# ChangUk/RecommenderSystems

Hardware: AMD Instinct MI355X
Metric: RWR seeds/sec + achieved HBM GB/s on 100M-edge bipartite graph, 1/2/4/8 GPUs (higher is better)
Workload: dtype f64

## Files before the change

### include/rwr.h

```cpp
#ifndef RWR_H
#define RWR_H

#include <stdint.h>

#ifdef __cplusplus
extern "C" {
#endif

#define RWR_VERSION_STRING "0.4.0"

enum {
    RWR_OK            = 0,
    RWR_E_INVALID     = 1,
    RWR_E_RANGE       = 2,
    RWR_E_NO_DEVICE   = 3,
    RWR_E_HIP         = 4,
    RWR_E_NOMEM       = 5,
    RWR_E_CAPACITY    = 6,
    RWR_E_UNSUPPORTED = 7
};

enum { RWR_NODE_UNDEFINED = 0, RWR_NODE_USER = 1, RWR_NODE_ITEM = 2, RWR_NODE_ETC = 3 };
enum { RWR_EDGE_UNDEFINED = 0, RWR_EDGE_LIKE = 1, RWR_EDGE_FRIENDSHIP = 2, RWR_EDGE_FOLLOW = 3,
       RWR_EDGE_MENTION = 4, RWR_EDGE_AUTHORSHIP = 5, RWR_EDGE_PURCHASE = 6, RWR_EDGE_ETC = 7 };
// ... 16 lines not shown
    int32_t reserved0;
} rwr_opts;

typedef struct rwr_stats {
    int32_t struct_size;
    int32_t n;
    int64_t nnz_raw;
    int64_t nnz;
    int32_t uniform;
    int32_t tile_seeds;
    int32_t tile_group;
    int32_t mode;
    double  build_ms;
    double  spmm_ms;
    int64_t spmm_launches;
    int64_t spmm_seed_steps;
    double  chain_ms;
    int64_t chain_launches;
    double  rank_ms;
    double  iterate_wall_ms;
    double  total_wall_ms;
    int64_t seeds_done;
    int64_t chain_redo_blocks;
    double  spmm_dense_ms;
    int64_t spmm_dense_launches;
    int64_t spmm_dense_seed_steps;
    int32_t uniform_path;
    int32_t reserved1;
    int64_t frontier_list_launches;
    int64_t rank_fused_groups;
    int64_t rank_fused_fallbacks;
    int64_t rank_pruned_rows;
    double  rank_bound_ms;
} rwr_stats;


const char *rwr_version(void);
int32_t rwr_device_count(void);
const char *rwr_last_error(void);

int32_t rwr_graph_create(int32_t n, const int64_t *node_id, const uint8_t *node_type,
                         const int64_t *rowptr , const int32_t *dst, const uint8_t *etype,
                         const double *w, const rwr_opts *opts , rwr_graph **out);
int32_t rwr_graph_destroy(rwr_graph *g);
int32_t rwr_graph_update_links(rwr_graph *g, int64_t count, const int64_t *link_index,
                               const uint8_t *etype , const double *w );
int32_t rwr_graph_append_links(rwr_graph *g, int64_t count, const int32_t *src, const int32_t *dst,
                               const uint8_t *etype, const double *w,
                               int64_t *new_index_out );
int32_t rwr_graph_size(const rwr_graph *g, int32_t *n, int64_t *nnz_raw, int64_t *nnz_explicit);
int32_t rwr_graph_get_normalized(rwr_graph *g, double *w_out , uint8_t *dangling_out );

int32_t rwr_recommend(rwr_graph *g, int32_t seed, float d, int32_t n_iter, int32_t top_n,
                      int64_t *out_id, double *out_score, int64_t *inout_count);

int32_t rwr_recommend_eval(rwr_graph *g, int32_t seed, float d, int32_t n_iter, const int64_t *test_ids,
                           int64_t n_test, int64_t *n_hits, double *sum_precision, int64_t *list_len);

int32_t rwr_recommend_eval_batch(rwr_graph *g, const int32_t *seeds, int32_t K, float d, int32_t n_iter,
                                 const int64_t *test_ptr, const int64_t *test_ids, int64_t *n_hits,
                                 double *sum_precision, int64_t *list_len);

typedef struct rwr_graph_desc {
    int32_t n_nodes;
    int32_t reserved0;
    const int64_t *node_id;
// ... 47 lines not shown
```

### recommendersystems_amd/_lib.py

```python
from __future__ import annotations

import ctypes as C
import os

_HERE = os.path.dirname(os.path.abspath(__file__))
LIB_PATH = os.path.join(_HERE, "librwr.so")

RWR_OK, RWR_E_INVALID, RWR_E_RANGE, RWR_E_NO_DEVICE, RWR_E_HIP, RWR_E_NOMEM, RWR_E_CAPACITY, RWR_E_UNSUPPORTED = range(8)
RWR_MODE_EXACT = 0
RWR_RUN_ITERATIONS, RWR_RUN_THRESHOLD, RWR_RUN_DEFAULT_THRESHOLD = 0, 1, 2

EXPORTS = [
    "rwr_version", "rwr_device_count", "rwr_last_error",
    "rwr_graph_create", "rwr_graph_update_links", "rwr_graph_append_links", "rwr_graph_destroy", "rwr_graph_size", "rwr_graph_get_normalized",
    "rwr_recommend", "rwr_recommend_eval", "rwr_recommend_eval_batch", "rwr_eval_graphs", "rwr_recommend_batch", "rwr_model_run", "rwr_model_deliver",
    "rwr_model_run_restart", "rwr_model_deliver_restart", "rwr_model_run_batch", "rwr_model_run_restart_batch",
    "rwr_recommend_restart_batch",
    "rwr_part_begin", "rwr_part_step", "rwr_part_local_step", "rwr_part_finish_step", "rwr_part_rank",
    "rwr_get_stats", "rwr_reset_stats",
]


class rwr_opts(C.Structure):
    _fields_ = [("struct_size", C.c_int32), ("device", C.c_int32), ("mode", C.c_int32),
                ("tile_seeds", C.c_int32), ("tile_group", C.c_int32), ("profile", C.c_int32),
                ("workspace_bytes", C.c_int64), ("seed_row_kernel", C.c_int32), ("reserved0", C.c_int32)]


class rwr_graph_desc(C.Structure):
    _fields_ = [("n_nodes", C.c_int32), ("reserved0", C.c_int32), ("node_id", C.POINTER(C.c_int64)),
                ("node_type", C.POINTER(C.c_uint8)), ("rowptr", C.POINTER(C.c_int64)), ("dst", C.POINTER(C.c_int32)),
                ("etype", C.POINTER(C.c_uint8)), ("w", C.POINTER(C.c_double))]


class rwr_stats(C.Structure):
    _fields_ = [("struct_size", C.c_int32), ("n", C.c_int32), ("nnz_raw", C.c_int64), ("nnz", C.c_int64),
                ("uniform", C.c_int32), ("tile_seeds", C.c_int32), ("tile_group", C.c_int32), ("mode", C.c_int32),
                ("build_ms", C.c_double), ("spmm_ms", C.c_double), ("spmm_launches", C.c_int64),
                ("spmm_seed_steps", C.c_int64), ("chain_ms", C.c_double), ("chain_launches", C.c_int64),
                ("rank_ms", C.c_double), ("iterate_wall_ms", C.c_double), ("total_wall_ms", C.c_double),
                ("seeds_done", C.c_int64), ("chain_redo_blocks", C.c_int64),
                ("spmm_dense_ms", C.c_double), ("spmm_dense_launches", C.c_int64), ("spmm_dense_seed_steps", C.c_int64),
                ("uniform_path", C.c_int32), ("reserved1", C.c_int32), ("frontier_list_launches", C.c_int64),
                ("rank_fused_groups", C.c_int64), ("rank_fused_fallbacks", C.c_int64),
                ("rank_pruned_rows", C.c_int64), ("rank_bound_ms", C.c_double)]


class RwrError(RuntimeError):
    def __init__(self, status: int, message: str):
        super().__init__(f"librwr status {status}: {message}")
        self.status = status


_lib = None


def load():
    global _lib
    if _lib is not None:
        return _lib
    if not os.path.exists(LIB_PATH):
        raise ImportError(f"{LIB_PATH} not found: build it with `python -c 'import __graft_entry__ as g; g.build()'` "
                          "(hipcc --offload-arch=gfx950); there is no CPU fallback")
    lib = C.CDLL(LIB_PATH)
    p = C.POINTER
    lib.rwr_version.restype = C.c_char_p
    lib.rwr_last_error.restype = C.c_char_p
    lib.rwr_device_count.restype = C.c_int32
    lib.rwr_graph_create.restype = C.c_int32
    lib.rwr_graph_create.argtypes = [C.c_int32, p(C.c_int64), p(C.c_uint8), p(C.c_int64), p(C.c_int32),
                                     p(C.c_uint8), p(C.c_double), p(rwr_opts), p(C.c_void_p)]
    lib.rwr_graph_update_links.restype = C.c_int32
    lib.rwr_graph_update_links.argtypes = [C.c_void_p, C.c_int64, p(C.c_int64), p(C.c_uint8), p(C.c_double)]
    lib.rwr_graph_append_links.restype = C.c_int32
    lib.rwr_graph_append_links.argtypes = [C.c_void_p, C.c_int64, p(C.c_int32), p(C.c_int32), p(C.c_uint8), p(C.c_double),
                                           p(C.c_int64)]
    lib.rwr_graph_destroy.restype = C.c_int32
    lib.rwr_graph_destroy.argtypes = [C.c_void_p]
# ... 62 lines not shown
```

### recommendersystems_amd/csrc/api.hip

```cpp
#include <stdarg.h>
#include <algorithm>
#include <cmath>
#include <mutex>
#include <vector>
#include <stdlib.h>
#include <string.h>

#include "engine.h"
#include "exclude_plan.h"

namespace rwr {

static thread_local char g_err[512] = "";

void set_error(const char *fmt, ...)
{
    va_list ap;
    va_start(ap, fmt);
    vsnprintf(g_err, sizeof(g_err), fmt, ap);
    va_end(ap);
}

static int usable_devices()
{
// ... 954 lines not shown
}

int32_t rwr_part_rank(rwr_graph *g, void *dev_x, int32_t top_n, int64_t *ids, double *scores, int32_t *counts)
{
    g_err[0] = 0;
    if (!g || !dev_x || !ids || !scores || !counts) { set_error("rwr_part_rank: NULL argument"); return RWR_E_INVALID; }
    RWR_BIND(g);
    return part_rank(g, (double *)dev_x, top_n, ids, scores, counts);
}

int32_t rwr_get_stats(rwr_graph *g, rwr_stats *out)
{
    if (!g || !out) { set_error("rwr_get_stats: NULL argument"); return RWR_E_INVALID; }
    size_t sz = out->struct_size > 0 ? (size_t)out->struct_size : sizeof(rwr_stats);
    if (sz > sizeof(rwr_stats)) sz = sizeof(rwr_stats);
    rwr_stats s = g->stats;
    s.struct_size = (int32_t)sz;
    memcpy(out, &s, sz);
    return RWR_OK;
}

int32_t rwr_reset_stats(rwr_graph *g)
{
    if (!g) { set_error("rwr_reset_stats: NULL argument"); return RWR_E_INVALID; }
    rwr_stats &s = g->stats;
    s.spmm_ms = s.chain_ms = s.rank_ms = s.iterate_wall_ms = s.total_wall_ms = 0;
    s.spmm_launches = s.spmm_seed_steps = s.chain_launches = s.seeds_done = s.chain_redo_blocks = 0;
    s.spmm_dense_ms = 0;
    s.spmm_dense_launches = s.spmm_dense_seed_steps = 0;
    s.frontier_list_launches = 0;
    s.rank_fused_groups = s.rank_fused_fallbacks = 0;
    s.rank_pruned_rows = 0;
    s.rank_bound_ms = 0;
    return RWR_OK;
}

}
```

### recommendersystems_amd/csrc/iterate.hip

```cpp
#include "iterate.h"

#include <climits>
#include <cstdlib>
#include <type_traits>

namespace rwr {

template <int G, bool VF>
__global__ __launch_bounds__(256) void k_spmm(int32_t n, const int64_t *__restrict__ in_ptr,
                                              const int32_t *__restrict__ in_src,
                                              const double *__restrict__ in_w,
                                              const int32_t *__restrict__ row_order, int32_t nrows,
                                              const double *__restrict__ X, double *__restrict__ Y,
                                              const int32_t *__restrict__ seeds, double c1, int skip_seed_row,
                                              const double *__restrict__ w_src, double *__restrict__ Zout)
{
    constexpr int RPW = WAVE / G;
    constexpr int U = 4;
    const int tile = blockIdx.y;
    const size_t toff = (size_t)tile * (size_t)n * G;
    X += toff;
    Y += toff;
    if (VF && Zout) Zout += toff;
    const int lane = threadIdx.x & (WAVE - 1);
// ... 405 lines not shown
    double acc = 0.0;
    for (size_t w0 = 0; w0 < nzw; w0 += WAVE) {
        const uint32_t word = (w0 + lane < nzw) ? bits[w0 + lane] : 0u;
        unsigned long long mask = __ballot(word != 0u);
        while (mask) {
            const int l = __builtin_ctzll(mask);
            mask &= mask - 1;
            uint32_t wv = (uint32_t)__builtin_amdgcn_readlane((int)word, l);
            while (wv) {
                const int b = __builtin_ctz(wv);
                wv &= wv - 1;
                const int32_t i = (int32_t)((w0 + l) * 32 + b);
                if (consumer && s >= 0) {
                    while (p < e && in_src[p] < i) ++p;
                    while (p < e && in_src[p] == i) { acc += termp[p]; ++p; }
                    const double xi = x[(size_t)i * G + k];
                    const double rw = c1 * xi;
                    acc += dangling[i] ? xi : (xi - rw);
                }
            }
        }
    }
    if (consumer && s >= 0) {
        Y[(size_t)tile * (size_t)n * G + (size_t)s * G + k] = acc;
        if (nz_out && acc != 0.0)
            atomicOr(&nz_out[(size_t)tile * nzw + ((uint32_t)s >> 5)], 1u << (s & 31));
    }
}

constexpr int CH3_NSW = 6;
constexpr int CH3_NST = CH3_NSW * WAVE;
constexpr int CH3_LPT = 16;
constexpr int CH3_CE = CH3_NST * CH3_LPT;
template <int G>
__global__ __launch_bounds__(WAVE + CH3_NST) void k_seed_chain_roles(
    int32_t n, const int64_t *__restrict__ in_ptr, const int32_t *__restrict__ in_src,
    const uint8_t *__restrict__ dangling, const double *__restrict__ X, double *__restrict__ Y,
    const int32_t *__restrict__ seeds, double c1, const int64_t *__restrict__ evoff,
    const double *__restrict__ evterm, uint32_t *__restrict__ nz_out, unsigned int *__restrict__ gate)
{
    if (threadIdx.x == 0 && gate) __hip_atomic_fetch_add(gate, 1u, __ATOMIC_RELAXED, __HIP_MEMORY_SCOPE_AGENT);
    constexpr int CR = CH3_CE / G;
    static_assert(CR % 32 == 0, "chunk rows must be a multiple of 32");
    extern __shared__ double rr[];
    const int tile = blockIdx.x;
    const double *x = X + (size_t)tile * (size_t)n * G;
    const int tid = threadIdx.x;
    const int64_t total = (int64_t)n * G;
    const int nchunks = (int)((total + CH3_CE - 1) / CH3_CE);

    if (tid >= WAVE) {
        const int st = tid - WAVE;
        double rega[CH3_LPT], regb[CH3_LPT];
        uint8_t dga[CH3_LPT], dgb[CH3_LPT];
#define CH3_LOAD(R, D, C)                                                       \
    {                                                                           \
        const int64_t base__ = (int64_t)(C) * CH3_CE;                           \
        _Pragma("unroll") for (int u = 0; u < CH3_LPT; ++u) {                   \
            int64_t el = base__ + (int64_t)u * CH3_NST + st;                    \
            el = el < total ? el : total - 1;                                   \
            R[u] = x[el];                                                       \
            D[u] = dangling[el / G];                                            \
        }                                                                       \
    }
#define CH3_STAGE(R, D, C)                                                                              \
    {                                                                                                   \
        const int64_t base__ = (int64_t)(C) * CH3_CE;                                                   \
        double *buf__ = rr + (size_t)((C) & 1) * CH3_CE;                                                \
        _Pragma("unroll") for (int u = 0; u < CH3_LPT; ++u) {                                           \
            const int off = u * CH3_NST + st;                                                           \
            const double xv = (base__ + off < total) ? R[u] : 0.0;   \
            const double rw = c1 * xv;                                                                  \
            buf__[off] = D[u] ? xv : (xv - rw);                                                         \
        }                                                                                               \
    }
        CH3_LOAD(rega, dga, 0)
        if (nchunks > 1) CH3_LOAD(regb, dgb, 1)
        for (int c = 0; c < nchunks; c += 2) {
            CH3_STAGE(rega, dga, c)
            if (c + 2 < nchunks) CH3_LOAD(rega, dga, c + 2)
            __builtin_amdgcn_fence(__ATOMIC_RELEASE, "workgroup", "local");
            __builtin_amdgcn_s_barrier();
            if (c + 1 < nchunks) {
                CH3_STAGE(regb, dgb, c + 1)
                if (c + 3 < nchunks) CH3_LOAD(regb, dgb, c + 3)
                __builtin_amdgcn_fence(__ATOMIC_RELEASE, "workgroup", "local");
                __builtin_amdgcn_s_barrier();
            }
        }
#undef CH3_LOAD
#undef CH3_STAGE
        return;
    }

    const bool consumer = tid < G;
    const int k = tid % G;
    int32_t s = -1;
    int64_t p = 0, e = 0;
    const int32_t *srcp = in_src;
    const double *termp = evterm;
    int32_t nxt = INT_MAX, raw_s = INT_MAX;
    double tcur = 0.0, raw_t = 0.0;
    bool has2 = false;
    if (consumer) {
        s = seeds[tile * G + k];
        if (s >= 0) {
            p = in_ptr[s];
            e = in_ptr[s + 1];
            termp = evterm + evoff[tile * G + k] - p;
            if (p < e) { nxt = srcp[p]; tcur = termp[p]; ++p; }
            if (p < e) { raw_s = srcp[p]; raw_t = termp[p]; has2 = true; ++p; }
        }
    }
    double acc = 0.0;
    __builtin_amdgcn_s_setprio(3);
    for (int c = 0; c < nchunks; ++c) {
        __builtin_amdgcn_s_barrier();
        __builtin_amdgcn_fence(__ATOMIC_ACQUIRE, "workgroup", "local");
// ... 92 lines not shown
    bool any = false;
    if (j >= lo && j < hi) {
        const double w = w_src[j];
        const size_t at = (size_t)(j - lo) * G;
        for (int k = 0; k < G; ++k) {
            const double xv = X[(size_t)j * G + k];
            const double rw = c1 * xv;
            Zs[at + k] = rw * w;
            any = any || xv != 0.0;
        }
    }
    const unsigned long long m = __ballot(any);
    const int lane = threadIdx.x & (WAVE - 1);
    if (lane == 0 && (uint32_t)m) nz[(uint64_t)j >> 5] = (uint32_t)m;
    if (lane == 32 && (uint32_t)(m >> 32)) nz[(uint64_t)j >> 5] = (uint32_t)(m >> 32);
}


static PlanInput read_plan_knobs()
{
    PlanInput v;
    const char *e;
    if ((e = getenv("RWR_SPMM"))) v.spmm = atoi(e);
    if ((e = RWR_TUNE_ENV("RWR_NZ_ITERS"))) v.nz_iters = atoi(e);
    if ((e = getenv("RWR_ACT_ITERS"))) v.act_iters = atoi(e);
    if ((e = RWR_TUNE_ENV("RWR_ACT_MIN_N"))) v.act_min_n = atol(e);
    if ((e = getenv("RWR_FRONTIER_LIST"))) v.frontier_list = atoi(e);
    if ((e = getenv("RWR_CHAIN"))) v.chain = atoi(e);
    if ((e = RWR_TUNE_ENV("RWR_SCAN_WORK"))) v.scan_work = atof(e);
    if ((e = RWR_TUNE_ENV("RWR_SCAN_SIDE"))) v.scan_side = atoi(e);
    if ((e = RWR_TUNE_ENV("RWR_GATE"))) v.gate = atoi(e);
    if ((e = getenv("RWR_TAIL_ROWS"))) v.tail_rows = atoi(e);
    if ((e = RWR_TUNE_ENV("RWR_CHAIN_SERIAL"))) v.two_streams = atoi(e) == 0;
    return v;
}
static const PlanInput &plan_knobs() { static const PlanInput k = read_plan_knobs(); return k; }

template <class F> static void bool_dispatch(F &&f) { f(); }
template <class F, class... B> static void bool_dispatch(F &&f, bool b, B... bs)
{
    bool_dispatch([&](auto... c) { if (b) f(std::true_type{}, c...); else f(std::false_type{}, c...); }, bs...);
}

template <int G>
static void launch_spmm_g(rwr_graph *g, int tg, const SpmmArgs &a, hipStream_t s)
{
    const bool vf = a.Zin != nullptr;
    const double *GS = vf ? a.Zin : a.X;
    const int skip = a.skip_seed_row;
    constexpr int RPW = WAVE / G;
    constexpr int CH = G > 16 ? 16 : G;
    if constexpr (G >= 8) {
        if (a.rows.kind == Rows::Frontier) {
            const int32_t *fl_rows = g->fl_rows.p, *fl_cnt = g->fl_rows.p + (size_t)tg * (size_t)g->n;
            const unsigned want = cdiv((size_t)g->n / 10 + 1, (size_t)RPW * 4);
            const unsigned gx = want < 1u ? 1u : want < 2048u ? want : 2048u;
            bool_dispatch([&](auto v) {
                hipLaunchKernelGGL((k_spmm_frontier<G, CH, decltype(v)::value>), dim3(gx, tg), dim3(256), 0, s, g->n, g->in_ptr.p,
                                   g->in_src.p, g->in_w.p, fl_rows, fl_cnt, GS, a.Y, a.seeds, a.c1, skip, a.nz_in, a.nz_out,
                                   g->w_src.p, a.Zout);
            }, vf);
            return;
        }
    }
    const bool listed = a.rows.kind == Rows::Tail;
    const int32_t *order = listed ? g->tail_rows[a.rows.level].p : g->row_order.p;
// ... 49 lines not shown
    hipLaunchKernelGGL(k_init_seeds, dim3(cdiv((size_t)tg * G, 64)), dim3(64), 0, s, g->n, tg, G, X, seeds, nz, Z, g->w_src.p, c1);
}
void launch_make_z(int64_t elems, int G, const double *X, double *Z, const double *w_src, double c1, hipStream_t s)
{
    hipLaunchKernelGGL(k_make_z, dim3(cdiv((size_t)elems, 256)), dim3(256), 0, s, elems, G, X, Z, w_src, c1);
}
void launch_make_z_nz(rwr_graph *g, int32_t lo, int32_t hi, int G, const double *X, double *Zs, double c1, uint32_t *nz,
                      hipStream_t s)
{
    const int64_t first = (int64_t)lo & ~(int64_t)63;
    hipLaunchKernelGGL(k_make_z_nz, dim3(cdiv((size_t)((int64_t)hi - first), 256)), dim3(256), 0, s, lo, hi, G, X, Zs, g->w_src.p,
                       c1, nz);
}
void launch_mark_active(rwr_graph *g, int G, int tg, const uint32_t *nz, uint32_t *act, const int32_t *seeds, int32_t *fl_rows,
                        int32_t *fl_cnt, hipStream_t s)
{
    const size_t nzw = ((size_t)g->n + 31) / 32;
    hipLaunchKernelGGL(k_mark_active, dim3(cdiv(nzw, 4), tg), dim3(256), 0, s, g->n, nz, act, g->rowptr.p, g->dst.p, g->etype.p,
                       G, seeds, fl_rows, fl_cnt);
}
template <int G>
static void launch_seed_terms(rwr_graph *g, int tg, const double *X, const int32_t *seeds, double c1,
                              const int64_t *evoff, hipStream_t s, const double *Zin, const uint32_t *nz = nullptr)
{
    const unsigned term_blocks = g->max_in_deg > 256 * 8 ? 8u : cdiv((size_t)(g->max_in_deg > 0 ? g->max_in_deg : 1), 256);
    bool_dispatch([&](auto v) {
        hipLaunchKernelGGL((k_seed_terms<G, decltype(v)::value>), dim3(term_blocks, tg * G), dim3(256), 0, s, g->n, g->in_ptr.p,
                           g->in_src.p, g->in_w.p, Zin ? Zin : X, seeds, c1, evoff, g->d_evterm.p, nz);
    }, Zin != nullptr);
}
template <int G>
static void launch_chain(rwr_graph *g, int tg, const double *X, double *Y, const int32_t *seeds, double c1,
                         const int64_t *evoff, uint32_t *nz_out, unsigned int *gate, hipStream_t s,
                         Chain kind, const uint32_t *nz_x)
{
    if (kind == Chain::Sparse) {
        hipLaunchKernelGGL(k_seed_chain_sparse<G>, dim3(tg), dim3(64), 0, s, g->n, g->in_ptr.p, g->in_src.p,
                           g->dangling.p, X, Y, seeds, c1, evoff, g->d_evterm.p, nz_x, nz_out, gate);
        return;
    }
    if (kind == Chain::Roles) {
        constexpr size_t smem = 2 * CH3_CE * sizeof(double);
        (void)hipFuncSetAttribute((const void *)k_seed_chain_roles<G>, hipFuncAttributeMaxDynamicSharedMemorySize, (int)smem);
        hipLaunchKernelGGL(k_seed_chain_roles<G>, dim3(tg), dim3(WAVE + CH3_NST), smem, s, g->n, g->in_ptr.p,
                           g->in_src.p, g->dangling.p, X, Y, seeds, c1, evoff, g->d_evterm.p, nz_out, gate);
        return;
    }
    hipLaunchKernelGGL(k_seed_chain<G>, dim3(cdiv((size_t)tg * G, 64)), dim3(64), 0, s, g->n, tg, g->in_ptr.p,
                       g->in_src.p, g->in_w.p, g->dangling.p, X, Y, seeds, c1, nz_out);
}

int32_t Profile::record(hipEvent_t &e, hipStream_t s)
{
    e = nullptr;
    if (!on) return RWR_OK;
    if (used == pool.size()) { RWR_HIP(hipEventCreate(&e)); pool.push_back(e); }
    e = pool[used++];
    RWR_HIP(hipEventRecord(e, s));
    return RWR_OK;
}
int32_t Profile::end(std::vector<hipEvent_t> &stage, hipEvent_t a, hipStream_t s)
{
    hipEvent_t b; RWR_TRY(record(b, s));
    if (on) stage.insert(stage.end(), {a, b});
    return RWR_OK;
}
int32_t Profile::fold(rwr_graph *g)
{
    auto drain = [&](const std::vector<hipEvent_t> &v, double *acc, bool dense_only) -> int32_t {
        for (size_t i = 0; i + 1 < v.size(); i += 2) {
            float ms = 0.f;
            if (dense_only && !dense[i / 2]) continue;
            RWR_HIP(hipEventElapsedTime(&ms, v[i], v[i + 1]));
            *acc += ms;
        }
        return RWR_OK;
    };
    if (on) {
        RWR_TRY(drain(spmm, &g->stats.spmm_dense_ms, true));
        RWR_TRY(drain(spmm, &g->stats.spmm_ms, false));
        RWR_TRY(drain(chain, &g->stats.chain_ms, false));
        RWR_TRY(drain(rank, &g->stats.rank_ms, false));
        RWR_TRY(drain(iter, &g->stats.iterate_wall_ms, false));
        RWR_TRY(drain(bound, &g->stats.rank_bound_ms, false));
    }
    reset();
    return RWR_OK;
}

int32_t GroupIter::init(bool fresh, bool ranks_nonneg, bool ranking_only)
{
    const int32_t n = g->n;
    hipStream_t s = g->stream;
    const size_t elems = (size_t)tg * (size_t)n * G;
    PlanInput in = plan_knobs();
    in.n = n; in.nnz = g->nnz; in.nonneg = g->nonneg; in.big_n = spmv_big_n(); in.seed_row_kernel = g->opts.seed_row_kernel;
    in.scan_self = chain_scan_self_contained(G); in.G = G; in.tg = tg; in.c1 = c1;
    in.fresh = fresh; in.ranks_nonneg = ranks_nonneg; in.ranking_only = ranking_only;
    cfg = plan_config(in);
    if (fresh) RWR_HIP(hipMemsetAsync(X, 0, elems * sizeof(double), s));
    if (!fresh && Zc) launch_make_z((int64_t)elems, G, X, Zc, g->w_src.p, c1, s);
    const size_t nzw = ((size_t)n + 31) / 32;
    if (cfg.flist && g->fl_rows.ensure((size_t)tg * (size_t)n + (size_t)tg) != RWR_OK) {
        (void)hipGetLastError();
        cfg.flist = false;
    }
    if (fresh && Zc && !cfg.flist) RWR_HIP(hipMemsetAsync(Zc, 0, elems * sizeof(double), s));
    nz_cur = cfg.nz_iters > 0 ? g->d_nz.p : nullptr;
    nz_oth = cfg.nz_iters > 0 ? g->d_nz.p + (size_t)tg * nzw : nullptr;
    if (nz_cur) RWR_HIP(hipMemsetAsync(nz_cur, 0, (size_t)tg * nzw * sizeof(uint32_t), s));
    if (fresh) launch_init_seeds(g, G, tg, X, d_seeds, nz_cur, Zc, c1, s);
    RWR_HIP(hipGetLastError());
    if (cfg.scan) RWR_TRY(chain_scan_prepare(g, G, tg, d_seeds, s));
    if (Zc && G == 1 && tg == 1 && cfg.addends_nonneg) RWR_TRY(sweep_prepare(g));
    if (Zc && cfg.chain_kind == 0 && !cfg.scan) RWR_TRY(ensure_in_w(g));
    return RWR_OK;
}

int32_t GroupIter::step(const StepPlan &p, Profile &prof, int32_t row_first, int32_t row_count)
{
    const int32_t n = g->n;
    hipStream_t s = g->stream;
    const size_t nzw = ((size_t)n + 31) / 32;
    constexpr int GATE_SLOTS = 64;
    const uint32_t *nz_in = p.probe ? nz_cur : nullptr;
    uint32_t *nz_out = p.write_bits ? nz_oth : nullptr;
    if (nz_out) RWR_HIP(hipMemsetAsync(nz_out, 0, (size_t)tg * nzw * sizeof(uint32_t), s));
    uint32_t *act = p.mark ? g->d_nz.p + 2 * (size_t)tg * nzw : nullptr;
    const bool listed = p.rows.kind == Rows::Frontier;
    if (act) {
        int32_t *fl_rows = listed ? g->fl_rows.p : nullptr, *fl_cnt = listed ? fl_rows + (size_t)tg * (size_t)n : nullptr;
        RWR_HIP(hipMemsetAsync(act, 0, (size_t)tg * nzw * sizeof(uint32_t), s));
        if (fl_cnt) RWR_HIP(hipMemsetAsync(fl_cnt, 0, (size_t)tg * sizeof(int32_t), s));
        launch_mark_active(g, G, tg, nz_in, act, d_seeds, fl_rows, fl_cnt, s);
    }
    const uint32_t *nz_terms = p.terms_nz ? nz_in : nullptr;
    double *zout = (Zc && p.form_z) ? Zn : nullptr;
    hipStream_t sc = p.chain_side ? g->stream2 : s;
    unsigned int *gate_it = p.gate ? g->d_gate.p + (it % GATE_SLOTS) : nullptr;
    if (p.chain != Chain::None) {
        if (!p.scan()) RWR_DISPATCH_G(G, launch_seed_terms<GG>(g, tg, X, d_seeds, c1, d_evoff, s, Zc, nz_terms));
        if (gate_it) RWR_HIP(hipMemsetAsync(gate_it, 0, sizeof(unsigned int), s));
        if (p.chain_side) { RWR_HIP(hipEventRecord(g->ev_fork, s)); RWR_HIP(hipStreamWaitEvent(sc, g->ev_fork, 0)); }
        if (p.scan() && !(p.chain_self && Zc)) RWR_DISPATCH_G(G, launch_seed_terms<GG>(g, tg, X, d_seeds, c1, d_evoff, sc, Zc, nz_terms));
        hipEvent_t c0; RWR_TRY(prof.record(c0, sc));
        if (p.scan())
            RWR_TRY(chain_scan_step(g, G, tg, X, Y, d_seeds, d_evoff, c1, nz_out, sc, p.chain_self ? Zc : nullptr,
                                    p.chain_self ? zout : nullptr));
        else
            RWR_DISPATCH_G(G, launch_chain<GG>(g, tg, X, Y, d_seeds, c1, d_evoff, nz_out, gate_it, sc, p.chain, nz_in));
        RWR_TRY(prof.end(prof.chain, c0, sc));
        if (p.chain_side) RWR_HIP(hipEventRecord(g->ev_join, sc));
    }
    if (gate_it) hipLaunchKernelGGL(k_gate, dim3(1), dim3(1), 0, s, gate_it, (unsigned)(tg < 192 ? tg : 192));
    hipEvent_t a; RWR_TRY(prof.record(a, s));
    SpmmArgs sp;
    sp.X = X, sp.Y = Y, sp.seeds = d_seeds, sp.c1 = c1, sp.skip_seed_row = true;
    sp.nz_in = nz_in, sp.nz_out = nz_out, sp.act = act, sp.Zin = Zc, sp.Zout = zout;
    sp.hub_scan = cfg.addends_nonneg, sp.rows = p.rows;
    sp.row_first = row_first, sp.row_count = row_count;
    launch_spmm(g, G, tg, sp, s);
    RWR_TRY(prof.end(prof.spmm, a, s));
    if (prof.on) prof.dense.push_back(p.dense());
    if (p.dense()) { g->stats.spmm_dense_launches += 1; ++dense_steps; }
    if (p.chain_side) RWR_HIP(hipStreamWaitEvent(s, g->ev_join, 0));
    if (zout && p.seed_z) hipLaunchKernelGGL(k_seed_z, dim3(cdiv((size_t)tg * G, 64)), dim3(64), 0, s, n, tg, G, Y, zout, d_seeds, g->w_src.p, c1);
    RWR_HIP(hipGetLastError());
    { double *t = X; X = Y; Y = t; }
    { double *t = Zc; Zc = Zn; Zn = t; }
    { uint32_t *tz = nz_cur; nz_cur = nz_oth; nz_oth = tz; }
    g->stats.spmm_launches += 1;
    g->stats.chain_launches += p.chain != Chain::None; g->stats.frontier_list_launches += listed;
    ++it;
    return RWR_OK;
}

int32_t GroupIter::redo_rows(const StepPlan &p, Profile &prof, int32_t row_first, int32_t row_count, const SelSink *sel)
{
    hipStream_t s = g->stream;
    hipEvent_t a; RWR_TRY(prof.record(a, s));
    SpmmArgs sp;
    sp.X = Y, sp.Y = X, sp.seeds = d_seeds, sp.c1 = c1, sp.skip_seed_row = true;
    sp.Zin = Zn, sp.Zout = nullptr;
    sp.hub_scan = cfg.addends_nonneg, sp.rows = p.rows;
    sp.row_first = row_first, sp.row_count = row_count, sp.sel = sel;
    launch_spmm(g, G, tg, sp, s);
    RWR_TRY(prof.end(prof.spmm, a, s));
    if (prof.on) prof.dense.push_back(0);
    RWR_HIP(hipGetLastError());
    return RWR_OK;
}

int32_t iterate_group(rwr_graph *g, int G, int tg, const int32_t *d_seeds, const int64_t *d_evoff, const int32_t *h_seeds,
                      double d, int64_t T, Profile &prof, double **final_X, int64_t *dense_steps, SplitLast *split)
{
    GroupIter gi(g, G, tg, d_seeds, d_evoff, d);
    RWR_TRY(gi.init(true, true, true));
    if (gi.cfg.tails) {
        RWR_TRY(tail_rows_prepare(g));
        gi.cfg.tail_depth = g->tail_depth;
        for (size_t q = 0; q < (size_t)tg * G; ++q)
            if (h_seeds[q] >= 0) gi.cfg.need |= g->h_tail_flag[h_seeds[q]];
    }
    bool split_ok = false;
    if (split && split->head > 0 && T >= 1 && G >= 8 && plan_knobs().spmm != 0) {
        const StepPlan last = plan_step(gi.cfg, T - 1, T);
        split_ok = last.rows.kind == Rows::Tail && last.rows.level == 0 && !last.probe && !last.write_bits && !last.form_z &&
                   last.chain == Chain::None;
        split->last = last;
    }
    while (gi.it < T) {
        const StepPlan p = plan_step(gi.cfg, gi.it, T);
        if (split_ok && gi.it == T - 1) RWR_TRY(gi.step(p, prof, 0, split->head));
        else RWR_TRY(gi.step(p, prof));
    }
    if (split_ok) { split->taken = true; split->gi.emplace(gi); }
    *final_X = gi.X;
    *dense_steps = gi.dense_steps;
    return RWR_OK;
}

}
```

### recommendersystems_amd/csrc/rank_fused.hip

```cpp
#include "iterate.h"
#include "rank_bound.h"
#include "rank_keys.h"

namespace rwr {

static_assert(FUSED_SORT_SLOTS == SEL_SLOTS, "rank_plan.h sizes the candidate capacity by the merge's sort slots");

__global__ void k_sel_tau(int nseg, int32_t top_n, const int32_t *__restrict__ slot_k, const int32_t *__restrict__ out_counts,
                          const double *__restrict__ out_score, double *__restrict__ tau, int32_t *__restrict__ cursor)
{
    const int q = blockIdx.x * blockDim.x + threadIdx.x;
    if (q >= nseg) return;
    const int32_t orow = slot_k[q];
    double t = 0.0;
    if (orow >= 0 && out_counts[orow] >= top_n) t = out_score[(size_t)orow * top_n + (top_n - 1)];
    tau[q] = t;
    cursor[q] = 0;
}

constexpr int MERGE_LIKES = 256;
__global__ __launch_bounds__(256) void k_sel_merge(const int32_t *__restrict__ slot_k, const int32_t *__restrict__ seeds,
                                                   int32_t top_n, const int32_t *__restrict__ cursor,
                                                   const RowScore *__restrict__ body, int32_t cap, int32_t stride,
                                                   const int64_t *__restrict__ rowptr, const int32_t *__restrict__ dst,
// ... 187 lines not shown
        }
        const int64_t deg = e - p;
        if (deg > BOUND_MAX_DEG) e = p;
        float acc = 0.0f;
        bool outside = false;
        while (__any(p < e)) {
            const int64_t left = e - p;
            const int cnt = left > BOUND_W ? BOUND_W : (left > 0 ? (int)left : 0);
            const int32_t my_idx = (k < cnt) ? in_src[p + k] : src_lo;
            for (int c0 = 0; c0 < BOUND_W; c0 += CH) {
                if (!__any(c0 < cnt)) break;
                float mv[CH];
#pragma unroll
                for (int t = 0; t < CH; ++t) {
                    const int idx = __builtin_amdgcn_ds_bpermute(gbase + ((c0 + t) << 2), my_idx);
                    const uint32_t u = (uint32_t)(idx - src_lo);
                    const bool in = u < (uint32_t)nsrc;
                    mv[t] = (c0 + t < cnt && in) ? m[(size_t)u * BOUND_W] : 0.0f;
                    if (c0 + t < cnt && !in) outside = true;
                }
#pragma unroll
                for (int t = 0; t < CH; ++t) acc += mv[t];
            }
            p += cnt;
        }
        const bool kp = real && (never || outside || !bound_prunes(acc, deg));
        const unsigned long long kb = __ballot(kp), sb = __ballot(real && !kp && r < nrows);
        if (k == 0 && r < nrows) keep[r] = (uint32_t)(kb >> (sub * BOUND_W));
        skipped += (unsigned long long)__popcll(sb);
    }
    if (lane == 0 && skipped) atomicAdd(pruned, skipped);
}

__global__ __launch_bounds__(256) void k_sel_bound_compact(const int32_t *__restrict__ rows, int32_t nrows,
                                                           const uint32_t *__restrict__ keep, int32_t *__restrict__ list,
                                                           int32_t *__restrict__ list_cnt)
{
    const int tile = blockIdx.y;
    const int lane = threadIdx.x & (WAVE - 1);
    const uint32_t *kw = keep + (size_t)(tile / BOUND_W) * (size_t)nrows;
    int32_t *out = list + (size_t)tile * (size_t)nrows;
    const int wpb = blockDim.x / WAVE;
    const int64_t nwaves = (int64_t)gridDim.x * wpb;
    for (int64_t b0 = ((int64_t)blockIdx.x * wpb + threadIdx.x / WAVE) * WAVE; b0 < nrows; b0 += nwaves * WAVE) {
        const int64_t q = b0 + lane;
        const bool kp = q < nrows && ((kw[q] >> (tile % BOUND_W)) & 1u);
        const unsigned long long bal = __ballot(kp);
        if (!bal) continue;
        int32_t base = 0;
        if (lane == 0) base = atomicAdd(&list_cnt[tile], (int32_t)__popcll(bal));
        base = __shfl(base, 0);
        if (kp) out[base + __popcll(bal & ((1ull << lane) - 1ull))] = rows[q];
    }
}

static int32_t rank_bound_prepare(rwr_graph *g, int G, int tg, const int32_t *d_seeds, const double *Z, int32_t first,
                                  int32_t count, SelSink *sink, unsigned long long **pruned, hipStream_t s)
{
    *pruned = nullptr;
    if (!rank_knobs().prune || !Z || count <= 0 || tg <= 0) return RWR_OK;
    const int32_t *rows = g->tail_rows[0].p + first;
    const size_t nblk = cdiv((size_t)tg, (size_t)BOUND_W);
    const size_t head_bytes = 256 + (((size_t)tg * 2 * sizeof(int32_t) + 255) & ~(size_t)255);
    const size_t keep_bytes = (nblk * (size_t)count * sizeof(uint32_t) + 255) & ~(size_t)255;
    auto give_up = [&]() { (void)hipGetLastError(); return RWR_OK; };
    if (g->bound_first != first) {
        if (g->bound_ws.ensure(head_bytes + keep_bytes) != RWR_OK) return give_up();
        int32_t *range = (int32_t *)(g->bound_ws.p + 8);
        const int32_t init[2] = {INT32_MAX, -1};
        int32_t got[2] = {0, 0};
        RWR_HIP(hipMemcpyAsync(range, init, sizeof init, hipMemcpyHostToDevice, s));
        hipLaunchKernelGGL(k_sel_bound_range, dim3((unsigned)(cdiv((size_t)count, 256) < 4096 ? cdiv((size_t)count, 256) : 4096)),
                           dim3(256), 0, s, g->in_ptr.p, g->in_src.p, rows, count, range);
        RWR_HIP(hipMemcpyAsync(got, range, sizeof got, hipMemcpyDeviceToHost, s));
        RWR_HIP(hipStreamSynchronize(s));
        g->bound_lo = got[1] >= 0 ? got[0] : 0;
        g->bound_hi = got[1] >= 0 ? got[1] + 1 : 0;
        g->bound_first = first;
    }
    const int32_t nsrc = g->bound_hi - g->bound_lo;
    if (nsrc <= 0) return RWR_OK;
    const size_t table_bytes = nblk * (size_t)nsrc * BOUND_W * sizeof(float);
    if (g->bound_ws.ensure(head_bytes + keep_bytes + table_bytes) != RWR_OK) return give_up();
    unsigned long long *d_pruned = (unsigned long long *)g->bound_ws.p;
    int32_t *noprune = (int32_t *)(g->bound_ws.p + 256);
    uint32_t *keep = (uint32_t *)(g->bound_ws.p + head_bytes);
    float *m = (float *)(g->bound_ws.p + head_bytes + keep_bytes);
    RWR_HIP(hipMemsetAsync(d_pruned, 0, sizeof(unsigned long long), s));
    hipLaunchKernelGGL(k_sel_bound_flags, dim3(cdiv((size_t)tg, 64)), dim3(64), 0, s, tg, G, d_seeds, sink->tau, noprune);
    const unsigned gt = (unsigned)(cdiv((size_t)nsrc, 4) < 65536 ? cdiv((size_t)nsrc, 4) : 65536);
    RWR_DISPATCH_G(G, {
        if constexpr (GG >= 8)
            hipLaunchKernelGGL(k_sel_bound_table<GG>, dim3(gt, (unsigned)nblk), dim3(256), 0, s, g->n, tg, g->bound_lo, nsrc, Z,
                               d_seeds, sink->tau, m);
    });
    const unsigned want = cdiv((size_t)count, (size_t)(WAVE / BOUND_W) * 4 * 4);
    hipLaunchKernelGGL(k_sel_bound_rows, dim3(want < 1u ? 1u : want < 16384u ? want : 16384u, (unsigned)nblk), dim3(256), 0, s, tg,
                       g->in_ptr.p, g->in_src.p, rows, count, g->bound_lo, nsrc, m, noprune, keep, d_pruned);
    RWR_HIP(hipGetLastError());
    if (g->fl_rows.ensure((size_t)tg * (size_t)count) != RWR_OK) return give_up();
    int32_t *list_cnt = noprune + tg;
    RWR_HIP(hipMemsetAsync(list_cnt, 0, (size_t)tg * sizeof(int32_t), s));
    const unsigned wc = cdiv((size_t)count, (size_t)WAVE * 4 * 4);
    hipLaunchKernelGGL(k_sel_bound_compact, dim3(wc < 1u ? 1u : wc < 4096u ? wc : 4096u, (unsigned)tg), dim3(256), 0, s, rows, count,
                       keep, g->fl_rows.p, list_cnt);
    RWR_HIP(hipGetLastError());
    sink->list = g->fl_rows.p, sink->list_cnt = list_cnt, sink->list_stride = count;
    *pruned = d_pruned;
    return RWR_OK;
}

int32_t rank_group_fused(rwr_graph *g, int G, int tg, const int32_t *d_slot_k, const int32_t *d_seeds, int32_t top_n, double *Xf,
                         SplitLast &split, Profile &prof, hipStream_t s, bool *ranked)
{
    const int32_t n_tail = g->tail_n[0];
    const int32_t H = split.head < n_tail ? split.head : n_tail;
    RWR_TRY(rank_group_select(g, G, tg, d_slot_k, top_n, Xf, d_seeds, s, g->tail_rows[0].p, H));
    *ranked = true;
    if (H < n_tail) {
        SelSink sink;
        RWR_TRY(rank_fused_prepare(g, G, tg, d_slot_k, top_n, &sink, s));
        unsigned long long *d_pruned = nullptr, pruned = 0;
        hipEvent_t b0; RWR_TRY(prof.record(b0, s));
        RWR_TRY(rank_bound_prepare(g, G, tg, d_seeds, split.gi->Zn, H, n_tail - H, &sink, &d_pruned, s));
        RWR_TRY(prof.end(prof.bound, b0, s));
        RWR_TRY(split.gi->redo_rows(split.last, prof, H, n_tail - H, &sink));
        RWR_TRY(rank_fused_merge(g, G, tg, d_slot_k, d_seeds, top_n, sink, s));
        int32_t overflow = 0;
        RWR_HIP(hipMemcpyAsync(&overflow, sink.overflow, sizeof(int32_t), hipMemcpyDeviceToHost, s));
        if (d_pruned) RWR_HIP(hipMemcpyAsync(&pruned, d_pruned, sizeof pruned, hipMemcpyDeviceToHost, s));
        RWR_HIP(hipStreamSynchronize(s));
        if (!overflow) g->stats.rank_pruned_rows += (int64_t)pruned;
        if (overflow) {
            RWR_TRY(split.gi->redo_rows(split.last, prof, 0, -1, nullptr));
            launch_exclude(g, G, tg, Xf, d_seeds, s);
            RWR_HIP(hipGetLastError());
            g->stats.rank_fused_fallbacks += 1;
            *ranked = false;
// ... 8 lines not shown
```

### recommendersystems_amd/csrc/step_plan.h

```cpp
#pragma once

#include <cstdint>

namespace rwr {

struct PlanInput {
    int spmm = 1, nz_iters = 4, act_iters = -1, frontier_list = 1, chain = 1;
    int64_t act_min_n = 200000; double scan_work = 10000.0;
    int scan_side = 1, gate = 1, tail_rows = 1;
    bool two_streams = true;
    int32_t n = 0, big_n = 2000000;
    int64_t nnz = 0; bool nonneg = true;
    int seed_row_kernel = 0;
    bool scan_self = false;
    int G = 1, tg = 1;
    double c1 = 0.85;
    bool fresh = true;
    bool ranks_nonneg = true;
    bool ranking_only = false;
};

struct PlanConfig {
    int G = 1, tg = 1; bool fresh = true;
    int nz_iters = 0;
    int act_iters = 0;
    bool flist = false;
    bool addends_nonneg = false;
    bool scan = false;
    int chain_kind = 1;
    bool scan_side = false, scan_self = false;
    bool two_streams = true, gate = true;
    bool tails = false; int tail_depth = 0;
    unsigned need = 0;
};

inline PlanConfig plan_config(const PlanInput &in)
{
    PlanConfig c;
    c.G = in.G, c.tg = in.tg, c.fresh = in.fresh;
    const bool single = in.G == 1 && in.tg == 1;
    c.nz_iters = (in.G >= 8 && in.spmm != 0 && in.nonneg) ? in.nz_iters : 0;
    c.act_iters = in.act_iters >= 0 ? in.act_iters : ((in.nnz / (in.n > 0 ? in.n : 1)) <= 64 ? 2 : 1);
    if (single && in.act_iters < 0 && c.act_iters == 2 && in.n >= in.big_n) c.act_iters = 3;
    if (single && in.spmm != 0 && in.nonneg) c.nz_iters = c.act_iters;
    if (single && in.act_iters < 0 && in.n < in.act_min_n) c.nz_iters = c.act_iters = 0;
    if (!in.fresh) c.nz_iters = c.act_iters = 0;
    c.flist = in.ranking_only && in.fresh && in.frontier_list != 0 && in.G >= 8 && c.nz_iters >= 2 && c.act_iters >= 1;
    c.chain_kind = in.seed_row_kernel == 1 ? 3 : in.seed_row_kernel == 2 ? 2 : in.seed_row_kernel == 3 ? 0 : in.chain;
    const double per_seed = 0.89 * (double)in.nnz / (double)(in.n > 0 ? in.n : 1) + 6.7;
    c.addends_nonneg = in.c1 >= 0.0 && in.c1 <= 1.0 && in.nonneg && in.ranks_nonneg;
    c.scan = c.addends_nonneg && (c.chain_kind == 2 || (c.chain_kind == 1 && (double)in.tg * in.G * per_seed < in.scan_work));
    c.scan_side = in.scan_side != 0 && single && in.two_streams && in.n >= 100000;
    c.scan_self = in.scan_self, c.two_streams = in.two_streams, c.gate = in.gate != 0;
    c.tails = in.ranking_only && in.tail_rows != 0 && !single;
    return c;
}

enum class Rows : uint8_t { All, Frontier, Tail };
struct RowSource { Rows kind = Rows::All; int level = 0; };
enum class Chain : uint8_t { None, Scan, ScanSide, Sparse, Roles, Simple };

struct StepPlan {
    RowSource rows;
    bool probe = false, write_bits = false;
    bool mark = false;
    bool terms_nz = false;
    Chain chain = Chain::None;
    bool chain_side = false, gate = false;
    bool chain_self = false;
    bool form_z = false, seed_z = false;
    bool dense() const { return !probe && rows.kind == Rows::All; }
    bool scan() const { return chain == Chain::Scan || chain == Chain::ScanSide; }
};

inline int last_tail(const PlanConfig &c)
{
    for (int k = 0; c.tails && k < c.tail_depth; ++k)
        if ((c.need >> k) & 1u) return k;
    return c.tails ? c.tail_depth - 1 : -1;
}

inline StepPlan plan_step(const PlanConfig &c, int64_t it, int64_t T)
{
    StepPlan p;
    const int64_t k = T - 1 - it;
    const bool last = T >= 0 && k == 0, tail = T >= 0 && k <= last_tail(c);
    p.probe = it < c.nz_iters;
    p.write_bits = it + 1 < c.nz_iters;
    p.mark = p.probe && it < c.act_iters;
    p.terms_nz = c.flist && p.probe;
    if (tail)
        p.rows = {Rows::Tail, (int)k};
    else if (c.flist && T >= 0 && !last && p.mark && p.write_bits && (it + 1 < c.act_iters || it == 1))
        p.rows = {Rows::Frontier, 0};
    if (tail && !((c.need >> k) & 1u)) p.chain = Chain::None;
    else if (c.scan && (!p.mark || c.G == 1)) p.chain = c.scan_side ? Chain::ScanSide : Chain::Scan;
    else if (p.mark) p.chain = Chain::Sparse;
    else p.chain = c.chain_kind == 0 ? Chain::Simple : Chain::Roles;
    const bool fold = p.chain != Chain::None && !p.scan();
    p.chain_side = p.chain == Chain::ScanSide || (fold && c.two_streams);
    p.gate = fold && c.two_streams && c.gate;
    p.chain_self = p.scan() && c.scan_self;
    p.form_z = !last;
    p.seed_z = p.form_z && p.chain != Chain::None && !p.chain_self;
    return p;
}

}
```

Baseline: 831.1.

## Skip fresh X memset under frontier lists and mask chain reads; rework bound compaction

On frontier-list plans, the initial hipMemsetAsync of X is skipped. The roles chain kernel instead takes a MASK template variant that reads the previous step's nonzero bitmap and treats rows not written by the frontier step as zero. The goal is to avoid a full clear of X, which costs an extra write pass over HBM per group. Separately, k_sel_bound_compact is rewritten to process all BOUND_W tiles of a block per pass, with one atomic per tile per span instead of one per wave, so the rows and keep arrays are read once rather than once per tile. This adds correctness risk: stale X values must never leak through unmasked reads. It also adds bitmap loads and extra register pressure in the chain kernel.

Result: faster. 839.5 (median of 6 runs) (+1.0%).

```diff
diff --git a/include/rwr.h b/include/rwr.h
--- a/include/rwr.h
+++ b/include/rwr.h
@@ -72,6 +72,7 @@
     int64_t rank_fused_fallbacks;
     int64_t rank_pruned_rows;
     double  rank_bound_ms;
+    int64_t x_clear_skipped;
 } rwr_stats;
 
 
diff --git a/recommendersystems_amd/_lib.py b/recommendersystems_amd/_lib.py
--- a/recommendersystems_amd/_lib.py
+++ b/recommendersystems_amd/_lib.py
@@ -43,7 +43,7 @@
                 ("spmm_dense_ms", C.c_double), ("spmm_dense_launches", C.c_int64), ("spmm_dense_seed_steps", C.c_int64),
                 ("uniform_path", C.c_int32), ("reserved1", C.c_int32), ("frontier_list_launches", C.c_int64),
                 ("rank_fused_groups", C.c_int64), ("rank_fused_fallbacks", C.c_int64),
-                ("rank_pruned_rows", C.c_int64), ("rank_bound_ms", C.c_double)]
+                ("rank_pruned_rows", C.c_int64), ("rank_bound_ms", C.c_double), ("x_clear_skipped", C.c_int64)]
 
 
 class RwrError(RuntimeError):
diff --git a/recommendersystems_amd/csrc/api.hip b/recommendersystems_amd/csrc/api.hip
--- a/recommendersystems_amd/csrc/api.hip
+++ b/recommendersystems_amd/csrc/api.hip
@@ -1010,7 +1010,8 @@
     s.rank_fused_groups = s.rank_fused_fallbacks = 0;
     s.rank_pruned_rows = 0;
     s.rank_bound_ms = 0;
-    return RWR_OK;
-}
-
-}
+    s.x_clear_skipped = 0;
+    return RWR_OK;
+}
+
+}
diff --git a/recommendersystems_amd/csrc/iterate.hip b/recommendersystems_amd/csrc/iterate.hip
--- a/recommendersystems_amd/csrc/iterate.hip
+++ b/recommendersystems_amd/csrc/iterate.hip
@@ -461,12 +461,13 @@
 constexpr int CH3_NST = CH3_NSW * WAVE;
 constexpr int CH3_LPT = 16;
 constexpr int CH3_CE = CH3_NST * CH3_LPT;
-template <int G>
+template <int G, bool MASK>
 __global__ __launch_bounds__(WAVE + CH3_NST) void k_seed_chain_roles(
     int32_t n, const int64_t *__restrict__ in_ptr, const int32_t *__restrict__ in_src,
     const uint8_t *__restrict__ dangling, const double *__restrict__ X, double *__restrict__ Y,
     const int32_t *__restrict__ seeds, double c1, const int64_t *__restrict__ evoff,
-    const double *__restrict__ evterm, uint32_t *__restrict__ nz_out, unsigned int *__restrict__ gate)
+    const double *__restrict__ evterm, uint32_t *__restrict__ nz_out, unsigned int *__restrict__ gate,
+    const uint32_t *__restrict__ nz_x)
 {
     if (threadIdx.x == 0 && gate) __hip_atomic_fetch_add(gate, 1u, __ATOMIC_RELAXED, __HIP_MEMORY_SCOPE_AGENT);
     constexpr int CR = CH3_CE / G;
@@ -477,12 +478,16 @@
     const int tid = threadIdx.x;
     const int64_t total = (int64_t)n * G;
     const int nchunks = (int)((total + CH3_CE - 1) / CH3_CE);
+    if (MASK) nz_x += (size_t)tile * (((size_t)n + 31) / 32);
 
     if (tid >= WAVE) {
         const int st = tid - WAVE;
         double rega[CH3_LPT], regb[CH3_LPT];
         uint8_t dga[CH3_LPT], dgb[CH3_LPT];
-#define CH3_LOAD(R, D, C)                                                       \
+        constexpr int NW = MASK ? CR / 32 : 1;
+        uint32_t bwa[NW], bwb[NW];
+        const int64_t nzw = ((int64_t)n + 31) / 32;
+#define CH3_LOAD(R, D, W, C)                                                    \
     {                                                                           \
         const int64_t base__ = (int64_t)(C) * CH3_CE;                           \
         _Pragma("unroll") for (int u = 0; u < CH3_LPT; ++u) {                   \
@@ -491,28 +496,44 @@
             R[u] = x[el];                                                       \
             D[u] = dangling[el / G];                                            \
         }                                                                       \
-    }
-#define CH3_STAGE(R, D, C)                                                                              \
+        if (MASK) {                                                             \
+            _Pragma("unroll") for (int j = 0; j < NW; ++j) {                    \
+                int64_t wi__ = (int64_t)(C) * (CR / 32) + j;                    \
+                wi__ = wi__ < nzw ? wi__ : nzw - 1;  \
+                W[j] = nz_x[wi__];                                              \
+            }                                                                   \
+        }                                                                       \
+    }
+#define CH3_STAGE(R, D, W, C)                                                                           \
     {                                                                                                   \
         const int64_t base__ = (int64_t)(C) * CH3_CE;                                                   \
         double *buf__ = rr + (size_t)((C) & 1) * CH3_CE;                                                \
         _Pragma("unroll") for (int u = 0; u < CH3_LPT; ++u) {                                           \
             const int off = u * CH3_NST + st;                                                           \
-            const double xv = (base__ + off < total) ? R[u] : 0.0;   \
+            bool live__ = base__ + off < total;                                                         \
+            if (MASK) {  \
+                const int row__ = off / G, j0__ = (u * CH3_NST / G) >> 5;                               \
+                uint32_t wd__ = W[j0__];                                                                \
+                _Pragma("unroll") for (int dj = 1; dj <= 2; ++dj)                                       \
+                    if (j0__ + dj < NW && (row__ >> 5) == j0__ + dj) wd__ = W[j0__ + dj < NW ? j0__ + dj : 0]; \
+                live__ = live__ && ((wd__ >> (row__ & 31)) & 1u);                                       \
+            }                                                                                           \
+            const double xv = live__ ? R[u] : 0.0;  \
             const double rw = c1 * xv;                                                                  \
             buf__[off] = D[u] ? xv : (xv - rw);                                                         \
         }                                                                                               \
     }
-        CH3_LOAD(rega, dga, 0)
-        if (nchunks > 1) CH3_LOAD(regb, dgb, 1)
+        static_assert(!MASK || (CH3_NST - 1) / G + 1 <= 64, "a thread's value of one load lies at most two bitmap words on");
+        CH3_LOAD(rega, dga, bwa, 0)
+        if (nchunks > 1) CH3_LOAD(regb, dgb, bwb, 1)
         for (int c = 0; c < nchunks; c += 2) {
-            CH3_STAGE(rega, dga, c)
-            if (c + 2 < nchunks) CH3_LOAD(rega, dga, c + 2)
+            CH3_STAGE(rega, dga, bwa, c)
+            if (c + 2 < nchunks) CH3_LOAD(rega, dga, bwa, c + 2)
             __builtin_amdgcn_fence(__ATOMIC_RELEASE, "workgroup", "local");
             __builtin_amdgcn_s_barrier();
             if (c + 1 < nchunks) {
-                CH3_STAGE(regb, dgb, c + 1)
-                if (c + 3 < nchunks) CH3_LOAD(regb, dgb, c + 3)
+                CH3_STAGE(regb, dgb, bwb, c + 1)
+                if (c + 3 < nchunks) CH3_LOAD(regb, dgb, bwb, c + 3)
                 __builtin_amdgcn_fence(__ATOMIC_RELEASE, "workgroup", "local");
                 __builtin_amdgcn_s_barrier();
             }
@@ -671,6 +692,7 @@
     if ((e = RWR_TUNE_ENV("RWR_GATE"))) v.gate = atoi(e);
     if ((e = getenv("RWR_TAIL_ROWS"))) v.tail_rows = atoi(e);
     if ((e = RWR_TUNE_ENV("RWR_CHAIN_SERIAL"))) v.two_streams = atoi(e) == 0;
+    if ((e = getenv("RWR_X_CLEAR"))) v.x_clear = atoi(e);
     return v;
 }
 static const PlanInput &plan_knobs() { static const PlanInput k = read_plan_knobs(); return k; }
@@ -786,7 +808,7 @@
 template <int G>
 static void launch_chain(rwr_graph *g, int tg, const double *X, double *Y, const int32_t *seeds, double c1,
                          const int64_t *evoff, uint32_t *nz_out, unsigned int *gate, hipStream_t s,
-                         Chain kind, const uint32_t *nz_x)
+                         Chain kind, const uint32_t *nz_x, bool masked)
 {
     if (kind == Chain::Sparse) {
         hipLaunchKernelGGL(k_seed_chain_sparse<G>, dim3(tg), dim3(64), 0, s, g->n, g->in_ptr.p, g->in_src.p,
@@ -795,9 +817,13 @@
     }
     if (kind == Chain::Roles) {
         constexpr size_t smem = 2 * CH3_CE * sizeof(double);
-        (void)hipFuncSetAttribute((const void *)k_seed_chain_roles<G>, hipFuncAttributeMaxDynamicSharedMemorySize, (int)smem);
-        hipLaunchKernelGGL(k_seed_chain_roles<G>, dim3(tg), dim3(WAVE + CH3_NST), smem, s, g->n, g->in_ptr.p,
-                           g->in_src.p, g->dangling.p, X, Y, seeds, c1, evoff, g->d_evterm.p, nz_out, gate);
+        bool_dispatch([&](auto m) {
+            constexpr bool MASK = decltype(m)::value && G >= 8;
+            (void)hipFuncSetAttribute((const void *)k_seed_chain_roles<G, MASK>, hipFuncAttributeMaxDynamicSharedMemorySize,
+                                      (int)smem);
+            hipLaunchKernelGGL((k_seed_chain_roles<G, MASK>), dim3(tg), dim3(WAVE + CH3_NST), smem, s, g->n, g->in_ptr.p,
+                               g->in_src.p, g->dangling.p, X, Y, seeds, c1, evoff, g->d_evterm.p, nz_out, gate, nz_x);
+        }, masked);
         return;
     }
     hipLaunchKernelGGL(k_seed_chain<G>, dim3(cdiv((size_t)tg * G, 64)), dim3(64), 0, s, g->n, tg, g->in_ptr.p,
@@ -852,13 +878,15 @@
     in.scan_self = chain_scan_self_contained(G); in.G = G; in.tg = tg; in.c1 = c1;
     in.fresh = fresh; in.ranks_nonneg = ranks_nonneg; in.ranking_only = ranking_only;
     cfg = plan_config(in);
-    if (fresh) RWR_HIP(hipMemsetAsync(X, 0, elems * sizeof(double), s));
     if (!fresh && Zc) launch_make_z((int64_t)elems, G, X, Zc, g->w_src.p, c1, s);
     const size_t nzw = ((size_t)n + 31) / 32;
     if (cfg.flist && g->fl_rows.ensure((size_t)tg * (size_t)n + (size_t)tg) != RWR_OK) {
         (void)hipGetLastError();
         cfg.flist = false;
-    }
+        cfg.clear_x = plan_clear_x(cfg);
+    }
+    if (fresh && cfg.clear_x) RWR_HIP(hipMemsetAsync(X, 0, elems * sizeof(double), s));
+    if (fresh && !cfg.clear_x) g->stats.x_clear_skipped += 1;
     if (fresh && Zc && !cfg.flist) RWR_HIP(hipMemsetAsync(Zc, 0, elems * sizeof(double), s));
     nz_cur = cfg.nz_iters > 0 ? g->d_nz.p : nullptr;
     nz_oth = cfg.nz_iters > 0 ? g->d_nz.p + (size_t)tg * nzw : nullptr;
@@ -902,7 +930,8 @@
             RWR_TRY(chain_scan_step(g, G, tg, X, Y, d_seeds, d_evoff, c1, nz_out, sc, p.chain_self ? Zc : nullptr,
                                     p.chain_self ? zout : nullptr));
         else
-            RWR_DISPATCH_G(G, launch_chain<GG>(g, tg, X, Y, d_seeds, c1, d_evoff, nz_out, gate_it, sc, p.chain, nz_in));
+            RWR_DISPATCH_G(G, launch_chain<GG>(g, tg, X, Y, d_seeds, c1, d_evoff, nz_out, gate_it, sc, p.chain, nz_in,
+                                                       p.chain_masked));
         RWR_TRY(prof.end(prof.chain, c0, sc));
         if (p.chain_side) RWR_HIP(hipEventRecord(g->ev_join, sc));
     }
@@ -949,7 +978,7 @@
                       double d, int64_t T, Profile &prof, double **final_X, int64_t *dense_steps, SplitLast *split)
 {
     GroupIter gi(g, G, tg, d_seeds, d_evoff, d);
-    RWR_TRY(gi.init(true, true, true));
+    RWR_TRY(gi.init(true, true, T >= 1));
     if (gi.cfg.tails) {
         RWR_TRY(tail_rows_prepare(g));
         gi.cfg.tail_depth = g->tail_depth;
diff --git a/recommendersystems_amd/csrc/rank_fused.hip b/recommendersystems_amd/csrc/rank_fused.hip
--- a/recommendersystems_amd/csrc/rank_fused.hip
+++ b/recommendersystems_amd/csrc/rank_fused.hip
@@ -243,25 +243,60 @@
     if (lane == 0 && skipped) atomicAdd(pruned, skipped);
 }
 
-__global__ __launch_bounds__(256) void k_sel_bound_compact(const int32_t *__restrict__ rows, int32_t nrows,
-                                                           const uint32_t *__restrict__ keep, int32_t *__restrict__ list,
-                                                           int32_t *__restrict__ list_cnt)
-{
-    const int tile = blockIdx.y;
-    const int lane = threadIdx.x & (WAVE - 1);
-    const uint32_t *kw = keep + (size_t)(tile / BOUND_W) * (size_t)nrows;
-    int32_t *out = list + (size_t)tile * (size_t)nrows;
-    const int wpb = blockDim.x / WAVE;
-    const int64_t nwaves = (int64_t)gridDim.x * wpb;
-    for (int64_t b0 = ((int64_t)blockIdx.x * wpb + threadIdx.x / WAVE) * WAVE; b0 < nrows; b0 += nwaves * WAVE) {
-        const int64_t q = b0 + lane;
-        const bool kp = q < nrows && ((kw[q] >> (tile % BOUND_W)) & 1u);
-        const unsigned long long bal = __ballot(kp);
-        if (!bal) continue;
-        int32_t base = 0;
-        if (lane == 0) base = atomicAdd(&list_cnt[tile], (int32_t)__popcll(bal));
-        base = __shfl(base, 0);
-        if (kp) out[base + __popcll(bal & ((1ull << lane) - 1ull))] = rows[q];
+constexpr int COMPACT_RPT = 8, COMPACT_WAVES = 4, COMPACT_SPAN = COMPACT_WAVES * WAVE * COMPACT_RPT;
+__global__ __launch_bounds__(COMPACT_WAVES * WAVE) void k_sel_bound_compact(int tg, const int32_t *__restrict__ rows, int32_t nrows,
+                                                                            const uint32_t *__restrict__ keep,
+                                                                            int32_t *__restrict__ list, int32_t *__restrict__ list_cnt)
+{
+    static_assert(BOUND_W <= WAVE, "one lane per tile of the block");
+    __shared__ int32_t wcnt[COMPACT_WAVES][BOUND_W];
+    const int blk = blockIdx.y;
+    const int lane = threadIdx.x & (WAVE - 1), wv = threadIdx.x / WAVE;
+    const uint32_t *kw = keep + (size_t)blk * (size_t)nrows;
+    const int64_t nspans = ((int64_t)nrows + COMPACT_SPAN - 1) / COMPACT_SPAN;
+    for (int64_t sp = blockIdx.x; sp < nspans; sp += gridDim.x) {
+        const int64_t q0 = sp * COMPACT_SPAN + (int64_t)wv * (WAVE * COMPACT_RPT) + lane;
+        uint32_t w[COMPACT_RPT];
+        int32_t id[COMPACT_RPT];
+#pragma unroll
+        for (int i = 0; i < COMPACT_RPT; ++i) {
+            const int64_t q = q0 + (int64_t)i * WAVE;
+            w[i] = q < nrows ? kw[q] : 0u;
+            id[i] = q < nrows ? rows[q] : 0;
+        }
+        int32_t mine = 0;
+        for (int t = 0; t < BOUND_W; ++t) {
+            int32_t c = 0;
+#pragma unroll
+            for (int i = 0; i < COMPACT_RPT; ++i) c += (int32_t)__popcll(__ballot((w[i] >> t) & 1u));
+            if (lane == t) mine = c;
+        }
+        if (lane < BOUND_W) wcnt[wv][lane] = mine;
+        __syncthreads();
+        if (threadIdx.x < BOUND_W) {
+            const int tile = blk * BOUND_W + (int)threadIdx.x;
+            int32_t c[COMPACT_WAVES], total = 0;
+#pragma unroll
+            for (int v = 0; v < COMPACT_WAVES; ++v) total += c[v] = wcnt[v][threadIdx.x];
+            int32_t at = (total && tile < tg) ? atomicAdd(&list_cnt[tile], total) : 0;
+#pragma unroll
+            for (int v = 0; v < COMPACT_WAVES; ++v) { wcnt[v][threadIdx.x] = at; at += c[v]; }
+        }
+        __syncthreads();
+        for (int t = 0; t < BOUND_W; ++t) {
+            const int tile = blk * BOUND_W + t;
+            if (tile >= tg) break;
+            int32_t *out = list + (size_t)tile * (size_t)nrows;
+            int32_t at = wcnt[wv][t];
+#pragma unroll
+            for (int i = 0; i < COMPACT_RPT; ++i) {
+                const bool kp = (w[i] >> t) & 1u;
+                const unsigned long long bal = __ballot(kp);
+                if (kp) out[at + __popcll(bal & ((1ull << lane) - 1ull))] = id[i];
+                at += (int32_t)__popcll(bal);
+            }
+        }
+        __syncthreads();
     }
 }
 
@@ -312,9 +347,9 @@
     if (g->fl_rows.ensure((size_t)tg * (size_t)count) != RWR_OK) return give_up();
     int32_t *list_cnt = noprune + tg;
     RWR_HIP(hipMemsetAsync(list_cnt, 0, (size_t)tg * sizeof(int32_t), s));
-    const unsigned wc = cdiv((size_t)count, (size_t)WAVE * 4 * 4);
-    hipLaunchKernelGGL(k_sel_bound_compact, dim3(wc < 1u ? 1u : wc < 4096u ? wc : 4096u, (unsigned)tg), dim3(256), 0, s, rows, count,
-                       keep, g->fl_rows.p, list_cnt);
+    const size_t wc = cdiv((size_t)count, (size_t)COMPACT_SPAN);
+    hipLaunchKernelGGL(k_sel_bound_compact, dim3((unsigned)(wc < 65536 ? wc : 65536), (unsigned)nblk), dim3(COMPACT_WAVES * WAVE), 0,
+                       s, tg, rows, count, keep, g->fl_rows.p, list_cnt);
     RWR_HIP(hipGetLastError());
     sink->list = g->fl_rows.p, sink->list_cnt = list_cnt, sink->list_stride = count;
     *pruned = d_pruned;
diff --git a/recommendersystems_amd/csrc/step_plan.h b/recommendersystems_amd/csrc/step_plan.h
--- a/recommendersystems_amd/csrc/step_plan.h
+++ b/recommendersystems_amd/csrc/step_plan.h
@@ -5,7 +5,7 @@
 namespace rwr {
 
 struct PlanInput {
-    int spmm = 1, nz_iters = 4, act_iters = -1, frontier_list = 1, chain = 1;
+    int spmm = 1, nz_iters = 4, act_iters = -1, frontier_list = 1, chain = 1, x_clear = 0;
     int64_t act_min_n = 200000; double scan_work = 10000.0;
     int scan_side = 1, gate = 1, tail_rows = 1;
     bool two_streams = true;
@@ -32,7 +32,11 @@
     bool two_streams = true, gate = true;
     bool tails = false; int tail_depth = 0;
     unsigned need = 0;
+    bool force_clear = false;
+    bool clear_x = true;
 };
+
+inline bool plan_clear_x(const PlanConfig &c) { return c.force_clear || !c.flist || c.scan || c.chain_kind == 0; }
 
 inline PlanConfig plan_config(const PlanInput &in)
 {
@@ -53,6 +57,8 @@
     c.scan_side = in.scan_side != 0 && single && in.two_streams && in.n >= 100000;
     c.scan_self = in.scan_self, c.two_streams = in.two_streams, c.gate = in.gate != 0;
     c.tails = in.ranking_only && in.tail_rows != 0 && !single;
+    c.force_clear = in.x_clear != 0;
+    c.clear_x = plan_clear_x(c);
     return c;
 }
 
@@ -66,6 +72,7 @@
     bool mark = false;
     bool terms_nz = false;
     Chain chain = Chain::None;
+    bool chain_masked = false;
     bool chain_side = false, gate = false;
     bool chain_self = false;
     bool form_z = false, seed_z = false;
@@ -80,6 +87,14 @@
     return c.tails ? c.tail_depth - 1 : -1;
 }
 
+inline bool step_lists(const PlanConfig &c, int64_t it, int64_t T)
+{
+    const int64_t k = T - 1 - it;
+    if (!c.flist || T < 0 || it < 0 || k <= 0 || k <= last_tail(c)) return false;
+    const bool write_bits = it + 1 < c.nz_iters, mark = it < c.nz_iters && it < c.act_iters;
+    return mark && write_bits && (it + 1 < c.act_iters || it == 1);
+}
+
 inline StepPlan plan_step(const PlanConfig &c, int64_t it, int64_t T)
 {
     StepPlan p;
@@ -91,12 +106,13 @@
     p.terms_nz = c.flist && p.probe;
     if (tail)
         p.rows = {Rows::Tail, (int)k};
-    else if (c.flist && T >= 0 && !last && p.mark && p.write_bits && (it + 1 < c.act_iters || it == 1))
+    else if (step_lists(c, it, T))
         p.rows = {Rows::Frontier, 0};
     if (tail && !((c.need >> k) & 1u)) p.chain = Chain::None;
     else if (c.scan && (!p.mark || c.G == 1)) p.chain = c.scan_side ? Chain::ScanSide : Chain::Scan;
     else if (p.mark) p.chain = Chain::Sparse;
     else p.chain = c.chain_kind == 0 ? Chain::Simple : Chain::Roles;
+    p.chain_masked = !c.clear_x && p.chain != Chain::None && p.chain != Chain::Sparse && step_lists(c, it - 1, T);
     const bool fold = p.chain != Chain::None && !p.scan();
     p.chain_side = p.chain == Chain::ScanSide || (fold && c.two_streams);
     p.gate = fold && c.two_streams && c.gate;
```
